# trnKhanh/medical-image-analysis

Hardware: AMD Instinct MI355X
Metric: training images/sec (whole node), UNet 512x512 1ch bs=32/GPU (higher is better)
Workload: dtype bf16; 1 GPU; UNet-2D channels [64, 128, 256, 512, 1024] 512x512 1ch, batch 32/GPU, instance norm, dropout 0.1, Dice+CE, Adam(wd 5e-4), clip 10 (cfg3); global_batch=32, parallelism=dp1

## Files before the change

include/mia_hip.h:

```cpp
#ifndef MIA_HIP_H
#define MIA_HIP_H
#include <stdint.h>
#ifdef __cplusplus
extern "C" {
#endif

#define MIA_F32 0
#define MIA_BF16 1

int mia_version(void);
const char* mia_last_error(void);

int mia_pack_weight(const float* src, void* dst, int dtype, int d0, int d1, int taps, int npad, int kpad,
                    int n_from_d0, void* stream);
int mia_pack_desc_bytes(void);
int mia_pack_weight_batch(const void* descs_dev, int count, int total_bricks, int max_taps, int dtype, void* stream);
int mia_relayout(const void* src, int src_dtype, void* dst, int dst_dtype, int n, int c, int64_t hw,
                 int64_t ssn, int64_t ssc, int64_t ssp, int64_t dsn, int64_t dsc, int64_t dsp, void* stream);
int mia_add(const void* a, const void* b, void* out, int dtype, int64_t n, void* stream);
int mia_dropout_mask(float* out, int64_t n, float keep, uint64_t seed, uint64_t offset, void* stream);
int mia_dropout_mask_dyn(float* out, int64_t n, float keep, const uint64_t* seed_base, uint64_t rel_offset, void* stream);
int mia_zero(void* p, int64_t bytes, void* stream);
int mia_gather_f32(const float* src, int64_t stride, float* dst, int n, void* stream);
int mia_colsum_workspace(int64_t p, int c);
// ... 16 lines not shown
#define MIA_CONV_FAM_FAST 1
#define MIA_CONV_FAM_S2_WIDE 2
#define MIA_CONV_FAM_CONV64 3
#define MIA_CONV_FAM_CONV64_DMA 4
#define MIA_CONV_FAM_CONV_BT 5
#define MIA_CONV_FAM_CONV_PW 6
#define MIA_CONV_FAM_NL 7
#define MIA_CONV_FAM_ACC 8
#define MIA_CONV_VAR_STATS 4
#define MIA_CONV_VAR_BIAS 8
int mia_conv_mma_family(int mode, int dtype, int c1, int c2, int o1, int o2, int npad, int kpad, int hout, int wout, int variant,
                        int split);
int mia_split_desc_bytes(void);
int mia_split_f16_batch(const void* descs_dev, int count, void* stream);
int mia_amax(const float* x, int64_t n, void* slot, int reset, void* stream);
int mia_widen_u8_i64(const void* src, void* dst, int64_t n, void* stream);
int mia_host_narrow_labels(const int64_t* src, uint8_t* dst, int64_t n, int threads);
int mia_host_copy(void* dst, const void* src, int64_t bytes, int threads);
int mia_amax_desc_bytes(void);
int mia_amax_batch(const void* descs_dev, int count, void* slots, void* stream);

int mia_conv_nl_supported(int mode, int dtype, int c1, int nout, int hout, int wout);
int mia_conv_mma_nl(int mode, int dtype, const void* y_in, int c1, const float* in_scale, const float* in_shift, float slope,
                    const void* wpack, int npad, int kpad, const float* bias, void* out, int nout, float* stat_partials,
                    int n, int hin, int win, int hout, int wout, void* stream);

int mia_conv_acc_supported(int mode, int dtype, int c1, int nout);
int mia_conv_mma_acc(int mode, int dtype, const void* in1, int c1, const void* wpack, int npad, int kpad, int flip_taps,
                     void* out_inout, int nout, int n, int hin, int win, int hout, int wout, const void* amax_in, const void* amax_w,
                     const void* wpack_split, void* stream);


int mia_stem_slabs(void);
int mia_stem_wgrad_workspace(int c0);
int mia_stem_fwd(const void* x, int x_dtype, const float* w, const float* bias, void* y, int dtype, float* stat_partials, int n,
                 int h, int wd, int c0, void* stream);
int mia_stem_wgrad(const void* x, int x_dtype, const void* dy, int dtype, float* workspace, float* grad, int n, int h, int wd,
                   int c0, int accumulate, void* stream);
int mia_stem_wgrad_fused(const void* x, int x_dtype, const void* dz, const void* y, int dtype, const float* scale,
                         const float* shift, const float* xa, const float* xb, const float* c1, const float* c2, float slope,
                         float* workspace, float* grad, int n, int h, int wd, int c0, int accumulate, void* stream);
int mia_stem_dgrad(const void* dy, int dtype, const float* w, float* dx, int n, int h, int wd, int c0, void* stream);

#define MIA_WGRAD_3S1 0
#define MIA_WGRAD_3S2 1
#define MIA_WGRAD_2S2 2
int mia_wgrad_target_blocks(int mode, int dtype);
int mia_wgrad_geometry(int mode, int dtype, int hy, int wy, int* tiles_y, int* tiles_x);
int mia_wgrad_plan(int mode, int dtype, int c1, int c2, int cdy, int npad, int hy, int* column_blocks, int* target_blocks, int* tile_h);
#define MIA_WGRAD_FAM_DMA96 0
#define MIA_WGRAD_FAM_BT 1
#define MIA_WGRAD_FAM_DMA 2
#define MIA_WGRAD_FAM_2WG 3
#define MIA_WGRAD_FAM_2WG_NL 4
#define MIA_WGRAD_FAM_TILE_FAST 5
#define MIA_WGRAD_FAM_F32_FAST 6
#define MIA_WGRAD_FAM_F32_NARROW 7
#define MIA_WGRAD_FAM_GENERIC 8
int mia_wgrad_family(int mode, int dtype, int c1, int c2, int cdy, int npad, int variant, int split);
int mia_conv_wgrad(int mode, int dtype, const void* x1, int c1, const void* x2, int c2, const void* dy, int cdy,
                   float* slabs, int ksplit, int npad, int kpad, int n, int hx, int wx, int hy, int wy, const void* amax_x1,
                   const void* amax_x2, const void* amax_dy, void* stream);
int mia_wgrad_nl_supported(int mode, int dtype, int c1, int cdy);
int mia_conv_wgrad_nl(int mode, int dtype, const void* y_in, int c1, const float* in_scale, const float* in_shift, float slope,
                      const void* dy, int cdy, float* slabs, int ksplit, int npad, int kpad, int n, int hx, int wx, int hy,
                      int wy, void* stream);
int mia_wgrad_reduce(const float* slabs, int ksplit, int taps, int npad, int kpad, float* grad, int nn, int kk,
                     int accumulate, void* stream);

#define MIA_NORM_INSTANCE 0
#define MIA_NORM_BATCH 1
int mia_norm_finalize(const float* partials, int n, int tiles, int c, int64_t hw, int mode, int training,
                      const float* drop_scale, const float* gamma, const float* beta, float eps, float momentum,
                      float* running_mean, float* running_var, long long* num_batches, float* xa, float* xb,
                      float* scale, float* shift, float* ysum, void* stream);
int mia_norm_stats(const void* y, int dtype, int n, int64_t hw, int c, int slabs, float* partials, void* stream);
int mia_norm_act_fwd(const void* y, void* z, int dtype, const float* scale, const float* shift, int n, int64_t hw, int c,
                     float slope, void* amax_out, void* stream);
int mia_norm_two_piece_ok(int dtype, int c);
int mia_norm_act_bwd(const void* dz, const void* dz2, const void* y, void* dy, int dtype, const float* scale, const float* shift,
                     const float* xa, const float* xb, const float* ysum, int n, int64_t hw, int c, int mode,
                     int fixed_stats, float slope, int slabs, float* partials, float* c1, float* c2, float* dgamma,
                     float* dbeta, float* dbias, int accumulate, void* amax_out, void* stream);
int mia_norm_bwd_sums(const void* dz, const void* dz2, const void* y, int dtype, const float* scale, const float* shift,
                      const float* xa, const float* xb, const float* ysum, int n, int64_t hw, int c, int mode,
                      int fixed_stats, float slope, int slabs, float* partials, float* c1, float* c2, float* dgamma,
                      float* dbeta, float* dbias, int accumulate, void* stream);

int mia_bn_sync_local_stats(const float* partials, int n, int tiles, int c, int64_t hw, const float* drop_scale, float* xa,
                            float* xb, float* local, void* stream);
int mia_norm_finalize_sync(const float* gathered, int world, int n, int c, int64_t hw, const float* drop_scale,
                           const float* gamma, const float* beta, float eps, float momentum, float* running_mean,
                           float* running_var, long long* num_batches, float* xa, float* xb, float* scale, float* shift,
                           float* ysum, void* stream);
int mia_norm_act_bwd_reduce(const void* dz, const void* dz2, const void* y, int dtype, const float* scale, const float* shift, const float* xa,
                            const float* xb, int n, int64_t hw, int c, float slope, int slabs, float* partials, float* c1,
                            float* c2, float* tot, void* stream);
int mia_norm_act_bwd_apply_sync(const void* dz, const void* dz2, const void* y, void* dy, int dtype, const float* scale, const float* shift,
                                const float* xa, const float* xb, const float* ysum, int n, int64_t hw, int c, float slope,
                                float* c1, float* c2, const float* group_tot, float* dgamma, float* dbeta, float* dbias,
                                int accumulate, void* amax_out, void* stream);

int mia_head_fwd(const void* x, int dtype, const float* w, const float* b, float* logits, int n, int64_t hw, int c0, int k1,
                 int64_t osn, int64_t osk, int64_t osp, void* stream);
int mia_head_bwd_workspace(int c0, int k1);
int mia_head_bwd(const float* dlogits, const void* x, int dtype, const float* w, void* dx, float* dw, float* db,
                 float* workspace, int n, int64_t hw, int c0, int k1, int64_t gsn, int64_t gsk, int64_t gsp, int accumulate,
                 void* stream);
#define MIA_LOSS_SOFTMAX 1
#define MIA_LOSS_DO_BG 2
#define MIA_LOSS_BATCH 4
#define MIA_LOSS_SQUARED 8
#define MIA_LOSS_DENSE 16
int mia_dice_ce_workspace(int nb, int k1, int slabs);
int mia_dice_ce_fwd(const float* logits, const long long* labels, int nb, int64_t hw, int k1, int64_t sn, int64_t sk,
                    int64_t sp, int flags, float smooth, float dice_w, float ce_w, int slabs, float* workspace, float* sums,
                    float* coef, float* out, int* bad_label, void* stream);
int mia_dice_ce_bwd(const float* logits, const long long* labels, const float* coef, const float* grad_out, float* dlogits,
                    int nb, int64_t hw, int k1, int64_t sn, int64_t sk, int64_t sp, int64_t gsn, int64_t gsk, int64_t gsp,
                    int flags, float dice_w, float ce_w, void* stream);

int mia_ds_loss_workspace(int nb, int k1, int slabs);
int mia_ds_loss_fwd(const float* z, const long long* labels, int nb, int h, int w, int factor, int k1, int64_t sn, int64_t sk,
                    int64_t sp, int flags, float smooth, float dice_w, float ce_w, int slabs, float* workspace, float* sums,
                    float* coef, float* out, int* bad_label, void* stream);
int mia_ds_loss_bwd(const float* z, const long long* labels, const float* coef, const float* grad_out, float* dz, int nb, int h,
                    int w, int factor, int k1, int64_t sn, int64_t sk, int64_t sp, int64_t gsn, int64_t gsk, int64_t gsp, int flags,
                    float dice_w, float ce_w, void* stream);

int mia_head_norm_eligible(int dtype, int n, int64_t hw, int c0, int k1);
int mia_head_norm_fwd(const void* y, int dtype, const float* scale, const float* shift, float slope, const float* w,
                      const float* b, float* logits, int n, int64_t hw, int c0, int k1, int64_t osn, int64_t osk, int64_t osp,
                      void* stream);
int mia_head_norm_wgrad(const float* dlogits, const void* y, int dtype, const float* scale, const float* shift, float slope,
                        float* dw, float* db, float* workspace, int n, int64_t hw, int c0, int k1, int64_t gsn, int64_t gsk,
                        int64_t gsp, int accumulate, void* stream);
int mia_norm_act_bwd_head(const float* dlogits, const float* w, int k1, int64_t gsn, int64_t gsk, int64_t gsp, const void* y,
                          void* dy, int dtype, const float* scale, const float* shift, const float* xa, const float* xb,
                          const float* ysum, int n, int64_t hw, int c, int mode, int fixed_stats, float slope, int slabs,
                          float* partials, float* c1, float* c2, float* dgamma, float* dbeta, float* dbias, int accumulate,
                          void* amax_out, void* stream);
int mia_head_w_supported(int dtype, int c, int k1);
int mia_norm_act_bwd_head_w(const float* dlogits, const float* w, int k1, int64_t gsn, int64_t gsk, int64_t gsp,
                            const void* y, void* dy, int dtype, const float* scale, const float* shift, const float* xa,
                            const float* xb, const float* ysum, int n, int64_t hw, int c, int mode, int fixed_stats,
                            float slope, int slabs, float* partials, float* c1, float* c2, float* dgamma, float* dbeta,
                            float* dbias, int accumulate, float* head_workspace, float* dw_head, float* db_head,
                            int accumulate_head, void* amax_out, void* stream);

#define MIA_SEGLOSS_SOFTMAX 1
#define MIA_SEGLOSS_DO_BG 2
#define MIA_SEGLOSS_BATCH 4
#define MIA_SEGLOSS_LABEL_U8 8
#define MIA_SEGLOSS_IGNORE 16
int mia_seg_loss_workspace(int nb, int k1, int slabs);
int mia_seg_loss_fwd(const float* logits, const void* labels, const float* class_w, int nb, int64_t hw, int k1, int64_t sn,
                     int64_t sk, int64_t sp, int flags, int64_t ignore_label, float smooth, float dice_w, float ce_w, int slabs,
                     float* workspace, float* coef, float* out, int64_t* counts, int* bad_label, void* stream);
int mia_seg_loss_bwd(const float* logits, const void* labels, const float* class_w, const float* coef, const float* grad_out,
                     float* dlogits, int nb, int64_t hw, int k1, int64_t sn, int64_t sk, int64_t sp, int64_t gsn, int64_t gsk,
                     int64_t gsp, int flags, int64_t ignore_label, void* stream);
int mia_topk_ce_workspace(int64_t n_pixels);
int mia_topk_ce_fwd(const float* logits, const void* labels, const float* class_w, int nb, int64_t hw, int k1, int64_t sn,
                    int64_t sk, int64_t sp, int flags, int64_t ignore_label, int64_t n_top, float* workspace, float* out,
                    int* bad_label, void* stream);
int mia_topk_ce_bwd(const float* logits, const void* labels, const float* class_w, const float* workspace, const float* grad_out,
// ... 162 lines not shown
```

medical-image-analysis_amd/csrc/norm.hip:

```cpp
#include "common.h"
#include "options.h"
#include <stdlib.h>

#define NORM_INSTANCE 0
#define NORM_BATCH 1

template <bool INST>
__global__ __launch_bounds__(1024) void norm_fwd_sum_kernel(const float* __restrict__ part, int tiles, int c, float* __restrict__ xa, float* __restrict__ xb,
                                    int64_t hw, const float* __restrict__ drop, const float* __restrict__ gamma,
                                    const float* __restrict__ beta, float eps, float* __restrict__ scale, float* __restrict__ shift,
                                    float* __restrict__ ysum) {
  __shared__ double sh1[16][17], sh2[16][17];
  const int cl = threadIdx.x & 15, tl = threadIdx.x >> 4;
  const int n = blockIdx.x, ch = blockIdx.y * 16 + cl;
  double s1 = 0.0, s2 = 0.0;
  if (ch < c) {
    typedef float f2_t __attribute__((ext_vector_type(2)));
    const f2_t* p = reinterpret_cast<const f2_t*>(part) + (size_t)n * tiles * c + ch;
    int t = tl;
    for (; t + 192 < tiles; t += 256) {
      const f2_t v0 = p[(size_t)t * c], v1 = p[(size_t)(t + 64) * c], v2 = p[(size_t)(t + 128) * c], v3 = p[(size_t)(t + 192) * c];
      s1 += (double)v0.x + (double)v1.x + (double)v2.x + (double)v3.x;
      s2 += (double)v0.y + (double)v1.y + (double)v2.y + (double)v3.y;
    }
// ... 289 lines not shown
  } while (0)

extern "C" int mia_norm_stats(const void* y, int dtype, int n, int64_t hw, int c, int slabs, float* partials, void* stream) {
  MIA_CHECK_ARG(y && partials && n > 0 && hw > 0 && c > 0 && slabs > 0, "mia_norm_stats: bad arguments");
  hipStream_t st = static_cast<hipStream_t>(stream);
  if (c % 32 == 0 && (reinterpret_cast<uintptr_t>(y) & 15) == 0 && (dtype == MIA_BF16 || dtype == MIA_F32)) {
    if (dtype == MIA_BF16)
      CRV(bf16_t, false, static_cast<const bf16_t*>(y), static_cast<const bf16_t*>(nullptr), static_cast<const bf16_t*>(nullptr), nullptr, nullptr, nullptr, nullptr, 0.f);
    else
      CRV(float, false, static_cast<const float*>(y), static_cast<const float*>(nullptr), static_cast<const float*>(nullptr), nullptr, nullptr, nullptr, nullptr, 0.f);
    MIA_LAUNCH_CHECK();
    return MIA_OK;
  }
  if (dtype == MIA_BF16)
    hipLaunchKernelGGL(norm_stats_kernel<bf16_t>, dim3(n * slabs, ceil_div(c, 256)), dim3(256), 512 * sizeof(float), st, static_cast<const bf16_t*>(y), hw, c, slabs, partials);
  else if (dtype == MIA_F32)
    hipLaunchKernelGGL(norm_stats_kernel<float>, dim3(n * slabs, ceil_div(c, 256)), dim3(256), 512 * sizeof(float), st, static_cast<const float*>(y), hw, c, slabs, partials);
  else { mia_set_error("mia_norm_stats: bad dtype"); return MIA_EARG; }
  MIA_LAUNCH_CHECK();
  return MIA_OK;
}

extern "C" int mia_amax(const float* x, int64_t n, void* slot, int reset, void* stream);
template <typename T> __device__ __forceinline__ void amax_fold(unsigned& m, const T* out) {
  if constexpr (sizeof(T) == 4) {
#pragma unroll
    for (int e = 0; e < Elem<T>::EPU; ++e) { const unsigned b = __builtin_bit_cast(unsigned, out[e]) & 0x7FFFFFFFu; m = b > m ? b : m; }
  }
}
__device__ __forceinline__ void amax_publish(unsigned m, unsigned* __restrict__ slot) {
  __shared__ unsigned blk;
  if (threadIdx.x == 0) blk = 0u;
  __syncthreads();
#pragma unroll
  for (int o = 32; o > 0; o >>= 1) { const unsigned t = (unsigned)__shfl_xor((int)m, o, 64); m = t > m ? t : m; }
  if ((threadIdx.x & 63) == 0 && m != 0u) atomicMax(&blk, m);
  __syncthreads();
  if (threadIdx.x == 0) {
    const unsigned b = blk;
    if (b > __hip_atomic_load(slot, __ATOMIC_RELAXED, __HIP_MEMORY_SCOPE_AGENT)) atomicMax(slot, b);
  }
}

template <typename T>
__global__ __launch_bounds__(256) void norm_act_fwd_stream_kernel(const T* __restrict__ y, T* __restrict__ z,
                                                                  const float* __restrict__ scale, const float* __restrict__ shift,
                                                                  int64_t hw, int c, int slabs, int upb, float slope,
                                                                  unsigned* __restrict__ amax) {
  constexpr int EPU = Elem<T>::EPU;
  const int n = blockIdx.x / slabs, s = blockIdx.x % slabs;
  const int lanes = 256 / upb;
  const int u = blockIdx.y * upb + threadIdx.x % upb, pl = threadIdx.x / upb;
  const bool live = u * EPU < c;
  if (!live && (sizeof(T) != 4 || amax == nullptr)) return;
  const int64_t per = (hw + slabs - 1) / slabs, r0 = s * per, r1 = live ? (r0 + per < hw ? r0 + per : hw) : r0;
  float sc[EPU], sf[EPU];
  unsigned am = 0;
#pragma unroll
  for (int e = 0; e < EPU; ++e) { sc[e] = live ? scale[(size_t)n * c + u * EPU + e] : 0.f; sf[e] = live ? shift[(size_t)n * c + u * EPU + e] : 0.f; }
  const size_t base = (size_t)n * hw * c + (size_t)u * EPU;
  auto body = [&](const u32x4& raw, int64_t r) {
    alignas(16) T in[EPU]; alignas(16) T out[EPU];
    *reinterpret_cast<u32x4*>(in) = raw;
#pragma unroll
    for (int e = 0; e < EPU; ++e) {
      const float v = sc[e] * Elem<T>::ld(in + e) + sf[e];
      out[e] = Elem<T>::cvt(v > 0.f ? v : v * slope);
    }
    amax_fold<T>(am, out);
    store_data_fence();
    *reinterpret_cast<u32x4*>(z + base + r * c) = *reinterpret_cast<const u32x4*>(out);
    store_data_pad();
  };
  auto ld = [&](int64_t rr) -> u32x4 { return *reinterpret_cast<const u32x4*>(y + base + rr * c); };
  int64_t r = r0 + pl;
  for (; r + 3 * lanes < r1; r += 4 * lanes) {
    const u32x4 a0 = ld(r), a1 = ld(r + lanes), a2 = ld(r + 2 * lanes), a3 = ld(r + 3 * lanes);
    body(a0, r); body(a1, r + lanes); body(a2, r + 2 * lanes); body(a3, r + 3 * lanes);
  }
  for (; r < r1; r += lanes) body(ld(r), r);
  if constexpr (sizeof(T) == 4) { if (amax != nullptr) amax_publish(am, amax); }
}

template <typename T, bool TWO = false>
__global__ __launch_bounds__(256) void norm_act_bwd_stream_kernel(const T* __restrict__ dz, const T* __restrict__ dz2,
                                                                  const T* __restrict__ y, T* __restrict__ dy,
                                                                  const float* __restrict__ scale, const float* __restrict__ shift,
                                                                  const float* __restrict__ xa, const float* __restrict__ xb,
                                                                  const float* __restrict__ c1, const float* __restrict__ c2,
                                                                  int64_t hw, int c, int slabs, int upb, float slope,
                                                                  unsigned* __restrict__ amax) {
  constexpr int EPU = Elem<T>::EPU;
  const int n = blockIdx.x / slabs, s = blockIdx.x % slabs;
  const int lanes = 256 / upb;
  const int u = blockIdx.y * upb + threadIdx.x % upb, pl = threadIdx.x / upb;
  const bool live = u * EPU < c;
  if (!live && (sizeof(T) != 4 || amax == nullptr)) return;
  const int64_t per = (hw + slabs - 1) / slabs, r0 = s * per, r1 = live ? (r0 + per < hw ? r0 + per : hw) : r0;
  float sc[EPU], sf[EPU], ka[EPU], kb[EPU];
  unsigned am = 0;
#pragma unroll
  for (int e = 0; e < EPU; ++e) {
    const size_t o = live ? (size_t)n * c + u * EPU + e : 0;
    sc[e] = scale[o]; sf[e] = shift[o];
    ka[e] = -sc[e] * c2[o] * xa[o];
    kb[e] = -sc[e] * (c1[o] + c2[o] * xb[o]);
  }
  const size_t base = (size_t)n * hw * c + (size_t)u * EPU;
  auto body = [&](const u32x4& graw, const u32x4& g2raw, const u32x4& yraw, int64_t r) {
    alignas(16) T gin[EPU]; alignas(16) T g2in[EPU]; alignas(16) T yin[EPU]; alignas(16) T out[EPU];
    *reinterpret_cast<u32x4*>(gin) = graw;
    *reinterpret_cast<u32x4*>(g2in) = g2raw;
    *reinterpret_cast<u32x4*>(yin) = yraw;
#pragma unroll
    for (int e = 0; e < EPU; ++e) {
      const float yv = Elem<T>::ld(yin + e);
      float g = Elem<T>::ld(gin + e);
      if (TWO) g += Elem<T>::ld(g2in + e);
      out[e] = Elem<T>::cvt(norm_bwd_dy(g, yv, sc[e], sf[e], ka[e], kb[e], slope));
    }
    amax_fold<T>(am, out);
    store_data_fence();
    *reinterpret_cast<u32x4*>(dy + base + r * c) = *reinterpret_cast<const u32x4*>(out);
    store_data_pad();
  };
  const u32x4 zero = u32x4{0u, 0u, 0u, 0u};
  auto ld = [&](const T* ptr, int64_t r) { return *reinterpret_cast<const u32x4*>(ptr + base + r * c); };
  int64_t r = r0 + pl;
  for (; r + lanes < r1; r += 2 * lanes) {
    const u32x4 g0 = ld(dz, r), h0 = TWO ? ld(dz2, r) : zero, y0 = ld(y, r);
    const u32x4 g1 = ld(dz, r + lanes), h1 = TWO ? ld(dz2, r + lanes) : zero, y1 = ld(y, r + lanes);
    body(g0, h0, y0, r); body(g1, h1, y1, r + lanes);
  }
  for (; r < r1; r += lanes) body(ld(dz, r), TWO ? ld(dz2, r) : zero, ld(y, r), r);
  if constexpr (sizeof(T) == 4) { if (amax != nullptr) amax_publish(am, amax); }
}

static void stream_geometry(int n, int64_t hw, int c, int epu, int* slabs, int* upb, int* gy) {
  const int upp = c / epu;
  int ub = 1;
  while (ub < upp && ub < 64) ub <<= 1;
  *upb = ub;
  *gy = (upp + ub - 1) / ub;
  const int lanes = 256 / ub;
  const int target = mia_options().stream_blocks;
  int64_t sl = target / ((int64_t)n * *gy);
  const int64_t maxsl = hw / (lanes * 8) > 0 ? hw / (lanes * 8) : 1;
  if (sl > maxsl) sl = maxsl;
  if (sl < 1) sl = 1;
  *slabs = (int)sl;
}

template <typename T, bool VEC>
__global__ void norm_act_fwd_kernel(const T* __restrict__ y, T* __restrict__ z, const float* __restrict__ scale,
                                    const float* __restrict__ shift, int64_t hw, int c, int64_t total_units, float slope) {
  constexpr int EPU = VEC ? Elem<T>::EPU : 1;
  const int upp = c / EPU;
  for (int64_t u = (int64_t)blockIdx.x * blockDim.x + threadIdx.x; u < total_units; u += (int64_t)gridDim.x * blockDim.x) {
    const int64_t pix = u / upp;
    const int ch = (int)(u - pix * upp) * EPU;
    const int n = (int)(pix / hw);
    const float* sc = scale + (size_t)n * c + ch;
    const float* sf = shift + (size_t)n * c + ch;
    if constexpr (VEC) {
      const u32x4 raw = *reinterpret_cast<const u32x4*>(y + u * EPU);
      alignas(16) T in[EPU]; alignas(16) T out[EPU];
      *reinterpret_cast<u32x4*>(in) = raw;
#pragma unroll
      for (int e = 0; e < EPU; ++e) {
        const float v = sc[e] * Elem<T>::ld(in + e) + sf[e];
        out[e] = Elem<T>::cvt(v > 0.f ? v : v * slope);
      }
      *reinterpret_cast<u32x4*>(z + u * EPU) = *reinterpret_cast<const u32x4*>(out);
    } else {
      const float v = sc[0] * Elem<T>::ld(y + u) + sf[0];
      Elem<T>::st(z + u, v > 0.f ? v : v * slope);
    }
  }
}

extern "C" int mia_norm_act_fwd(const void* y, void* z, int dtype, const float* scale, const float* shift, int n, int64_t hw,
                                int c, float slope, void* amax_out, void* stream) {
  MIA_CHECK_ARG(y && z && scale && shift && n > 0 && hw > 0 && c > 0, "mia_norm_act_fwd: bad arguments");
  if (dtype != MIA_F32) amax_out = nullptr;
  const int epu = dtype == MIA_BF16 ? 8 : 4;
  const bool vec = (c % epu == 0) && ((reinterpret_cast<uintptr_t>(y) | reinterpret_cast<uintptr_t>(z)) & 15) == 0;
  const int64_t units = (int64_t)n * hw * (vec ? c / epu : c);
  const int blocks = (int)((units + 255) / 256 < 16384 ? (units + 255) / 256 : 16384);
  hipStream_t st = static_cast<hipStream_t>(stream);
// ... 130 lines not shown
  }
}

template <typename T, bool VEC>
__global__ void norm_act_bwd_apply_kernel(const T* __restrict__ dz, const T* __restrict__ y, T* __restrict__ dy,
                                          const float* __restrict__ scale, const float* __restrict__ shift,
                                          const float* __restrict__ xa, const float* __restrict__ xb,
                                          const float* __restrict__ c1, const float* __restrict__ c2, int64_t hw, int c,
                                          int64_t total_units, float slope) {
  constexpr int EPU = VEC ? Elem<T>::EPU : 1;
  const int upp = c / EPU;
  for (int64_t u = (int64_t)blockIdx.x * blockDim.x + threadIdx.x; u < total_units; u += (int64_t)gridDim.x * blockDim.x) {
    const int64_t pix = u / upp;
    const int ch = (int)(u - pix * upp) * EPU;
    const size_t o = (size_t)(pix / hw) * c + ch;
    alignas(16) T gin[EPU]; alignas(16) T yin[EPU]; alignas(16) T out[EPU];
    if constexpr (VEC) {
      *reinterpret_cast<u32x4*>(gin) = *reinterpret_cast<const u32x4*>(dz + u * EPU);
      *reinterpret_cast<u32x4*>(yin) = *reinterpret_cast<const u32x4*>(y + u * EPU);
    } else { gin[0] = dz[u]; yin[0] = y[u]; }
#pragma unroll
    for (int e = 0; e < EPU; ++e) {
      const float yv = Elem<T>::ld(yin + e);
      float g = Elem<T>::ld(gin + e);
      if (!(scale[o + e] * yv + shift[o + e] > 0.f)) g *= slope;
      const float xh = xa[o + e] * yv + xb[o + e];
      out[e] = Elem<T>::cvt(scale[o + e] * (g - c1[o + e] - xh * c2[o + e]));
    }
    if constexpr (VEC) *reinterpret_cast<u32x4*>(dy + u * EPU) = *reinterpret_cast<const u32x4*>(out);
    else dy[u] = out[0];
  }
}

static bool bwd_vec_ok(const void* dz, const void* y, const void* dy, int dtype, int c) {
  const int epu = dtype == MIA_BF16 ? 8 : 4;
  return (c % epu == 0) &&
         ((reinterpret_cast<uintptr_t>(y) | reinterpret_cast<uintptr_t>(dz) | reinterpret_cast<uintptr_t>(dy)) & 15) == 0;
}

struct NormBwd {
  const void *dz, *dz2, *y; void* dy; int dtype;
  const float *scale, *shift, *xa, *xb, *ysum;
  int n; int64_t hw; int c, mode, fixed_stats; float slope; int slabs;
  float *partials, *c1, *c2, *dgamma, *dbeta, *dbias; int accumulate;
  void* amax_out; hipStream_t st;
};

extern "C" int mia_norm_two_piece_ok(int dtype, int c) { return (dtype == MIA_BF16 || dtype == MIA_F32) && c % 32 == 0; }

static int bwd_check(const char* who, const NormBwd& p, bool tensors, bool need_partials, bool need_grads) {
  MIA_CHECK_ARG(tensors && p.scale && p.shift && p.xa && p.xb && p.c1 && p.c2 && (!need_partials || p.partials) &&
                (!need_grads || (p.dgamma && p.dbeta)), "%s: null pointer", who);
  MIA_CHECK_ARG(p.n > 0 && p.hw > 0 && p.c > 0 && (!need_partials || p.slabs > 0), "%s: bad shape", who);
  MIA_CHECK_ARG(p.dtype == MIA_BF16 || p.dtype == MIA_F32, "%s: bad dtype", who);
  MIA_CHECK_ARG(p.dz2 == nullptr || (p.c % 32 == 0 && bwd_vec_ok(p.dz, p.y, p.dy, p.dtype, p.c) && (reinterpret_cast<uintptr_t>(p.dz2) & 15) == 0),
                "%s: two-piece gradient needs c %% 32 == 0 and aligned tensors", who);
  return MIA_OK;
}

static void bwd_reduce_launch(const NormBwd& p) {
  const int n = p.n, c = p.c, slabs = p.slabs;
  const int64_t hw = p.hw; float* partials = p.partials; hipStream_t st = p.st;
  const bool vec = bwd_vec_ok(p.dz, p.y, nullptr, p.dtype, c);
#define RD(T) hipLaunchKernelGGL(norm_act_bwd_reduce_kernel<T>, dim3(n * slabs, ceil_div(c, 256)), dim3(256), 512 * sizeof(float), st,   \
                                 static_cast<const T*>(p.dz), static_cast<const T*>(p.y), p.scale, p.shift, p.xa, p.xb, hw, c, slabs, \
                                 p.slope, partials)
#define RDV(T) CRV(T, true, static_cast<const T*>(p.dz), static_cast<const T*>(p.y), static_cast<const T*>(p.dz2), p.scale, p.shift, p.xa, p.xb, p.slope)
  if (vec && c % 32 == 0) { if (p.dtype == MIA_BF16) RDV(bf16_t); else RDV(float); }
  else if (p.dtype == MIA_BF16) RD(bf16_t); else RD(float);
#undef RDV
#undef RD
}

static void bwd_finalize_launch(const NormBwd& p, bool producer_parts = false, const float* group_tot = nullptr) {
  const bool own = !producer_parts && group_tot == nullptr;
  const bool inline_sums = own && (int64_t)p.n * p.slabs <= 1024;
  if (group_tot == nullptr && !inline_sums)
    hipLaunchKernelGGL(norm_bwd_sum_kernel, dim3(p.n, ceil_div(p.c, 16)), dim3(256), 0, p.st, p.partials, p.slabs, p.c, p.c1, p.c2);
  hipLaunchKernelGGL(norm_bwd_finalize_kernel, dim3(ceil_div(p.c, 16)), dim3(256), 0, p.st, p.n, p.c, p.hw, p.mode, p.fixed_stats,
                     p.scale, p.xa, p.xb, p.ysum, p.c1, p.c2, p.dgamma, p.dbeta, p.dbias, p.accumulate, group_tot,
                     inline_sums ? p.partials : nullptr, own ? p.slabs : 0);
}

static void bwd_apply_launch(const NormBwd& p) {
  void* amax_out = p.dtype == MIA_F32 ? p.amax_out : nullptr;
  const int epu = p.dtype == MIA_BF16 ? 8 : 4;
  const bool vec = bwd_vec_ok(p.dz, p.y, p.dy, p.dtype, p.c);
  const int64_t units = (int64_t)p.n * p.hw * (vec ? p.c / epu : p.c);
  const int blocks = (int)((units + 255) / 256 < 16384 ? (units + 255) / 256 : 16384);
#define AP(T, V) hipLaunchKernelGGL((norm_act_bwd_apply_kernel<T, V>), dim3(blocks), dim3(256), 0, p.st,                   \
                                    static_cast<const T*>(p.dz), static_cast<const T*>(p.y), static_cast<T*>(p.dy), p.scale, p.shift, \
                                    p.xa, p.xb, p.c1, p.c2, p.hw, p.c, units, p.slope)
  if (vec) {
    int sl, upb, gy;
    stream_geometry(p.n, p.hw, p.c, epu, &sl, &upb, &gy);
#define BS(T, TWOF) hipLaunchKernelGGL((norm_act_bwd_stream_kernel<T, TWOF>), dim3(p.n * sl, gy), dim3(256), 0, p.st, static_cast<const T*>(p.dz), \
                                       static_cast<const T*>(p.dz2), static_cast<const T*>(p.y), static_cast<T*>(p.dy), p.scale, p.shift, p.xa, p.xb, \
                                       p.c1, p.c2, p.hw, p.c, sl, upb, p.slope, static_cast<unsigned*>(amax_out))
    if (p.dtype == MIA_BF16) { if (p.dz2) BS(bf16_t, true); else BS(bf16_t, false); }
    else { if (p.dz2) BS(float, true); else BS(float, false); }
#undef BS
  } else {
    if (p.dtype == MIA_BF16) AP(bf16_t, false);
    else AP(float, false);
    if (amax_out) (void)mia_amax(static_cast<const float*>(p.dy), (int64_t)p.n * p.hw * p.c, amax_out, 0, p.st);
  }
#undef AP
}

extern "C" int mia_norm_act_bwd(const void* dz, const void* dz2, const void* y, void* dy, int dtype, const float* scale, const float* shift,
                                const float* xa, const float* xb, const float* ysum, int n, int64_t hw, int c, int mode,
                                int fixed_stats, float slope, int slabs, float* partials, float* c1, float* c2, float* dgamma,
                                float* dbeta, float* dbias, int accumulate, void* amax_out, void* stream) {
  const NormBwd p{dz, dz2, y, dy, dtype, scale, shift, xa, xb, ysum, n, hw, c, mode, fixed_stats, slope, slabs, partials, c1, c2,
                  dgamma, dbeta, dbias, accumulate, amax_out, static_cast<hipStream_t>(stream)};
  if (int e = bwd_check("mia_norm_act_bwd", p, dz && y && dy, true, true)) return e;
  bwd_reduce_launch(p);
  bwd_finalize_launch(p);
  bwd_apply_launch(p);
  MIA_LAUNCH_CHECK();
  return MIA_OK;
}

extern "C" int mia_norm_bwd_sums(const void* dz, const void* dz2, const void* y, int dtype, const float* scale, const float* shift,
                                 const float* xa, const float* xb, const float* ysum, int n, int64_t hw, int c, int mode,
                                 int fixed_stats, float slope, int slabs, float* partials, float* c1, float* c2, float* dgamma,
                                 float* dbeta, float* dbias, int accumulate, void* stream) {
  const NormBwd p{dz, dz2, y, nullptr, dtype, scale, shift, xa, xb, ysum, n, hw, c, mode, fixed_stats, slope, slabs, partials, c1, c2,
                  dgamma, dbeta, dbias, accumulate, nullptr, static_cast<hipStream_t>(stream)};
  if (int e = bwd_check("mia_norm_bwd_sums", p, dz && y, true, true)) return e;
  bwd_reduce_launch(p);
  bwd_finalize_launch(p);
  MIA_LAUNCH_CHECK();
  return MIA_OK;
}

#ifdef MIA_EXPERIMENTS
extern "C" int mia_norm_act_bwd_pre(const void* dz, const void* y, void* dy, int dtype, const float* scale, const float* shift,
                                    const float* xa, const float* xb, const float* ysum, int n, int64_t hw, int c, int mode,
                                    int fixed_stats, float slope, int parts, const float* partials, float* c1, float* c2,
                                    float* dgamma, float* dbeta, float* dbias, int accumulate, void* amax_out, void* stream) {
  const NormBwd p{dz, nullptr, y, dy, dtype, scale, shift, xa, xb, ysum, n, hw, c, mode, fixed_stats, slope, parts,
                  const_cast<float*>(partials), c1, c2, dgamma, dbeta, dbias, accumulate, amax_out, static_cast<hipStream_t>(stream)};
  if (int e = bwd_check("mia_norm_act_bwd_pre", p, true, true, true)) return e;
  MIA_CHECK_ARG(dy == nullptr || (dz && y), "mia_norm_act_bwd_pre: the apply pass needs dz and y");
  bwd_finalize_launch(p, true);
  if (dy != nullptr) bwd_apply_launch(p);
  MIA_LAUNCH_CHECK();
  return MIA_OK;
}

#endif

__global__ void bn_bwd_local_tot_kernel(int n_img, int c, int64_t hw, const float* __restrict__ c1, const float* __restrict__ c2,
                                        float* __restrict__ tot) {
  __shared__ double sh1[16][17], sh2[16][17];
  const int cl = threadIdx.x & 15, tl = threadIdx.x >> 4;
  const int ch = blockIdx.x * 16 + cl;
  double tg = 0.0, tgx = 0.0;
  if (ch < c)
    for (int n = tl; n < n_img; n += 16) { tg += c1[(size_t)n * c + ch]; tgx += c2[(size_t)n * c + ch]; }
  sh1[tl][cl] = tg; sh2[tl][cl] = tgx;
  __syncthreads();
  if (tl == 0 && ch < c) {
    tg = 0.0; tgx = 0.0;
    for (int j = 0; j < 16; ++j) { tg += sh1[j][cl]; tgx += sh2[j][cl]; }
    tot[ch] = (float)tg; tot[c + ch] = (float)tgx; tot[2 * c + ch] = (float)((double)n_img * (double)hw);
  }
}

extern "C" int mia_norm_act_bwd_reduce(const void* dz, const void* dz2, const void* y, int dtype, const float* scale, const float* shift,
                                       const float* xa, const float* xb, int n, int64_t hw, int c, float slope, int slabs,
                                       float* partials, float* c1, float* c2, float* tot, void* stream) {
  const NormBwd p{dz, dz2, y, nullptr, dtype, scale, shift, xa, xb, nullptr, n, hw, c, NORM_BATCH, 0, slope, slabs, partials, c1, c2,
                  nullptr, nullptr, nullptr, 0, nullptr, static_cast<hipStream_t>(stream)};
  if (int e = bwd_check("mia_norm_act_bwd_reduce", p, dz && y && tot, true, false)) return e;
  bwd_reduce_launch(p);
  hipLaunchKernelGGL(norm_bwd_sum_kernel, dim3(n, ceil_div(c, 16)), dim3(256), 0, p.st, partials, slabs, c, c1, c2);
  hipLaunchKernelGGL(bn_bwd_local_tot_kernel, dim3(ceil_div(c, 16)), dim3(256), 0, p.st, n, c, hw, c1, c2, tot);
  MIA_LAUNCH_CHECK();
  return MIA_OK;
}

extern "C" int mia_norm_act_bwd_apply_sync(const void* dz, const void* dz2, const void* y, void* dy, int dtype, const float* scale,
                                           const float* shift, const float* xa, const float* xb, const float* ysum, int n,
                                           int64_t hw, int c, float slope, float* c1, float* c2, const float* group_tot,
                                           float* dgamma, float* dbeta, float* dbias, int accumulate, void* amax_out, void* stream) {
  const NormBwd p{dz, dz2, y, dy, dtype, scale, shift, xa, xb, ysum, n, hw, c, NORM_BATCH, 0, slope, 0, nullptr, c1, c2,
                  dgamma, dbeta, dbias, accumulate, amax_out, static_cast<hipStream_t>(stream)};
  if (int e = bwd_check("mia_norm_act_bwd_apply_sync", p, dz && y && dy && group_tot, false, true)) return e;
  bwd_finalize_launch(p, false, group_tot);
  bwd_apply_launch(p);
  MIA_LAUNCH_CHECK();
  return MIA_OK;
}

template <typename T, int K1, int CG, bool HWG = false>
__global__ __launch_bounds__(256) void colreduce_head_kernel(const float* __restrict__ dl, const float* __restrict__ w,
                                                             const T* __restrict__ y, const float* __restrict__ scale,
                                                             const float* __restrict__ shift, const float* __restrict__ xa,
                                                             const float* __restrict__ xb, int hw, int c, int slabs, float slope,
                                                             int64_t gsn, int64_t gsp, int64_t gsk, float* __restrict__ part, float* __restrict__ wpart) {
// ... 242 lines not shown
```

medical-image-analysis_amd/mia_hip/ops.py:

```python
from __future__ import annotations

import ctypes
import math
from typing import Optional, Tuple

import torch

from . import (BF16, CONV_G1, CONV_G2S2, CONV_G3S1, CONV_G3S2, CONV_T2S2, CONV_T3S2, F32, LOSS_BATCH, LOSS_DO_BG,
               LOSS_DENSE, LOSS_SOFTMAX, LOSS_SQUARED, NORM_BATCH, NORM_INSTANCE, REGLOSS_BATCH, REGLOSS_DO_BG, REGLOSS_IGNORE,
               REGLOSS_INDEX, REGLOSS_TARGET_U8, SEGLOSS_BATCH, SEGLOSS_DO_BG, SEGLOSS_IGNORE,
               SEGLOSS_LABEL_U8, SEGLOSS_SOFTMAX, WGRAD_2S2, WGRAD_3S1, WGRAD_3S2, MiaError, call, lib)

LRELU_SLOPE = 0.01
_c_int, _c_float, _c_i64 = ctypes.c_int, ctypes.c_float, ctypes.c_int64


def _p(t: Optional[torch.Tensor]):
    return None if t is None else ctypes.c_void_p(t.data_ptr())


def _stream():
    return ctypes.c_void_p(torch.cuda.current_stream().cuda_stream)


# ... 589 lines not shown


_BN_TRACKING = True


class no_bn_tracking:

    def __enter__(self):
        global _BN_TRACKING
        self._was, _BN_TRACKING = _BN_TRACKING, False

    def __exit__(self, *exc):
        global _BN_TRACKING
        _BN_TRACKING = self._was
        return False


def _norm_finalize(ctx, cfg: NormCfg, stats, gamma, beta, y) -> torch.Tensor:
    n, h, w, cout = y.shape
    hw = h * w
    coefs = torch.empty((5, n, cout), device=y.device, dtype=torch.float32)
    ctx.sync = sync = cfg.sync if (cfg.sync is not None and cfg.mode == NORM_BATCH and cfg.training and cfg.sync.world > 1) else None
    track = _BN_TRACKING or not cfg.training
    rmean, rvar, nbatch = (cfg.running_mean, cfg.running_var, cfg.num_batches) if track else (None, None, None)
    if sync is None:
        call("mia_norm_finalize", _p(stats), n, 0 if stats is None else stats.shape[1], cout, _c_i64(hw), cfg.mode, int(cfg.training),
             _p(cfg.drop_scale), _p(gamma.detach()), _p(beta.detach()), _c_float(cfg.eps), _c_float(cfg.momentum),
             _p(rmean), _p(rvar), _p(nbatch), _p(coefs[0]), _p(coefs[1]), _p(coefs[2]),
             _p(coefs[3]), _p(coefs[4]), _stream())
        return coefs
    local = torch.empty((3, cout), device=stats.device, dtype=torch.float32)
    call("mia_bn_sync_local_stats", _p(stats), n, stats.shape[1], cout, _c_i64(hw), _p(cfg.drop_scale), _p(coefs[0]),
         _p(coefs[1]), _p(local), _stream())
    gathered = sync.all_gather(local)
    call("mia_norm_finalize_sync", _p(gathered), sync.world, n, cout, _c_i64(hw), _p(cfg.drop_scale), _p(gamma.detach()),
         _p(beta.detach()), _c_float(cfg.eps), _c_float(cfg.momentum), _p(rmean), _p(rvar),
         _p(nbatch), _p(coefs[0]), _p(coefs[1]), _p(coefs[2]), _p(coefs[3]), _p(coefs[4]), _stream())
    return coefs


def _norm_act_fwd(y, scale, shift, slope) -> torch.Tensor:
    n, h, w, c = y.shape
    z = torch.empty_like(y)
    call("mia_norm_act_fwd", _p(y), _p(z), _dt(y), _p(scale), _p(shift), n, _c_i64(h * w), c, _c_float(slope), _p(_amax_new(z)), _stream())
    return z


class LazyAct:
    __slots__ = ("y", "coefs", "slope")

    def __init__(self, y, coefs, slope):
        self.y, self.coefs, self.slope = y, coefs, slope

    @property
    def shape(self):
        return self.y.shape

    @property
    def dtype(self):
        return self.y.dtype

    @property
    def device(self):
        return self.y.device

    def materialize(self) -> torch.Tensor:
        return LazyMaterializeFn.apply(self.y, self.coefs, self.slope)


class LazyMaterializeFn(torch.autograd.Function):

    @staticmethod
    def forward(ctx, y, coefs, slope):
        return _norm_act_fwd(y, coefs[2], coefs[3], slope)

    @staticmethod
    def backward(ctx, dz):
        return dz, None, None


FUSE_HEAD_W = __import__('os').environ.get('MIA_FUSE_HEAD_W', '1') != '0'
FUSE_STEM_BWD = __import__('os').environ.get('MIA_FUSE_STEM_BWD', '1') != '0'
FUSE_NL = __import__('os').environ.get('MIA_FUSE_NL', '1') != '0'


def nl_supported(dtype, cin: int, cout: int, h: int, w: int, train: bool) -> bool:
    if not FUSE_NL or dtype != torch.bfloat16:
        return False
    if not lib().mia_conv_nl_supported(CONV_G3S1, BF16, cin, cout, h, w):
        return False
    return (not train) or bool(lib().mia_wgrad_nl_supported(WGRAD_3S1, BF16, cin, cout))


class _NormBwd:

    def __init__(self, y, coefs, mode, fixed, slope, dests=None):
        self.y, self.coefs, self.mode, self.fixed, self.slope = y, coefs, mode, fixed, slope
        n, h, w, c = y.shape
        self.dtype, self.n, self.hw, self.c, self.slabs = _dt(y), n, h * w, c, _slabs_for(h * w)
        self.part = torch.empty((n, self.slabs, c, 2), device=y.device, dtype=torch.float32)
        self.cc = torch.empty((2, n, c), device=y.device, dtype=torch.float32)
        dgb = torch.empty((3, c), device=y.device, dtype=torch.float32)
        got = (None,) * 3 if dests is None else [grad_dest(p) for p in dests]
        self.dgamma, self.dbeta, self.dbias = (dgb[i] if g is None else g for i, g in enumerate(got))

    def _run(self, slabs, part):
        k = self.coefs
        return (_p(k[2]), _p(k[3]), _p(k[0]), _p(k[1]), _p(None if self.fixed else k[4]), self.n, _c_i64(self.hw), self.c, self.mode,
                int(self.fixed), _c_float(self.slope), slabs, _p(part), _p(self.cc[0]), _p(self.cc[1]), _p(self.dgamma),
                _p(self.dbeta), _p(self.dbias), 0)

    def plain(self, dz, dz2, dy) -> None:
        call("mia_norm_act_bwd", _p(dz), _p(dz2), _p(self.y), _p(dy), self.dtype, *self._run(self.slabs, self.part),
             _p(_amax_new(dy)), _stream())

    def sums(self, dz, dz2) -> None:
        call("mia_norm_bwd_sums", _p(dz), _p(dz2), _p(self.y), self.dtype, *self._run(self.slabs, self.part), _stream())

    def pre(self, parts, dz, dy) -> None:
        call("mia_norm_act_bwd_pre", _p(None if dy is None else dz), _p(None if dy is None else self.y), _p(dy), self.dtype,
             *self._run(parts.shape[1], parts), _p(None if dy is None else _amax_new(dy)), _stream())

    def synced(self, sync: BatchSync, dz, dz2, dy) -> None:
        k, cc = self.coefs, self.cc
        tot = torch.empty((3, self.c), device=self.y.device, dtype=torch.float32)
        call("mia_norm_act_bwd_reduce", _p(dz), _p(dz2), _p(self.y), self.dtype, _p(k[2]), _p(k[3]), _p(k[0]), _p(k[1]), self.n,
             _c_i64(self.hw), self.c, _c_float(self.slope), self.slabs, _p(self.part), _p(cc[0]), _p(cc[1]), _p(tot), _stream())
        sync.all_reduce_sum(tot)
        call("mia_norm_act_bwd_apply_sync", _p(dz), _p(dz2), _p(self.y), _p(dy), self.dtype, _p(k[2]), _p(k[3]), _p(k[0]), _p(k[1]),
             _p(k[4]), self.n, _c_i64(self.hw), self.c, _c_float(self.slope), _p(cc[0]), _p(cc[1]), _p(tot), _p(self.dgamma),
             _p(self.dbeta), _p(self.dbias), 0, _p(_amax_new(dy)), _stream())

    def run(self, dz, dz2, sync, on_load: bool) -> Optional[torch.Tensor]:
        pre = _take_cr(dz) if (dz2 is None and sync is None) else None
        dy = None if on_load else torch.empty_like(self.y)
        if pre is not None:
            self.pre(pre, dz, dy)
        elif sync is not None:
            self.synced(sync, dz, dz2, dy)
        elif on_load:
            self.sums(dz, dz2)
        else:
            self.plain(dz, dz2, dy)
        return dy

    def head(self, dl, st, w2, dy, entry="mia_norm_act_bwd_head", extra=()) -> None:
        call(entry, _p(dl), _p(w2), w2.shape[0], _c_i64(st[0]), _c_i64(st[1]), _c_i64(st[2]), _p(self.y), _p(dy), self.dtype,
             *self._run(self.slabs, self.part), *extra, _p(_amax_new(dy)), _stream())

    def head_w(self, dl, st, w2, dy, ws, dwh, dbh) -> None:
        self.head(dl, st, w2, dy, "mia_norm_act_bwd_head_w", (_p(ws), _p(dwh), _p(dbh), 0))


def _block_wgrad(nb: _NormBwd, x1, x2, weight, stride: int, nl, dy, stem: bool = False, dz=None, dz2=None) -> torch.Tensor:
    cout, cin = weight.shape[:2]
    y, k = nb.y, nb.coefs
    if not stem:
        dw = conv_wgrad(WGRAD_3S2 if stride == 2 else WGRAD_3S1, x1, x2, dy, weight.shape, cout, cin, out=grad_dest(weight), nl=nl)
    else:
        if dy is None and dz2 is not None:
            dz = dz + dz2
        ws = torch.empty(lib().mia_stem_wgrad_workspace(cout), device=y.device, dtype=torch.float32)
        dw = grad_dest(weight)
        if dw is None:
            dw = torch.empty(weight.shape, device=y.device, dtype=torch.float32)
        if dy is None:
            call("mia_stem_wgrad_fused", _p(x1), _dt(x1), _p(dz), _p(y), nb.dtype, _p(k[2]), _p(k[3]), _p(k[0]), _p(k[1]),
                 _p(nb.cc[0]), _p(nb.cc[1]), _c_float(nb.slope), _p(ws), _p(dw), nb.n, y.shape[1], y.shape[2], cout, 0, _stream())
        else:
            call("mia_stem_wgrad", _p(x1), _dt(x1), _p(dy), nb.dtype, _p(ws), _p(dw), nb.n, y.shape[1], y.shape[2], cout, 0, _stream())
    return dw


def _stem_dgrad(dy, weight, x1) -> torch.Tensor:
    n, h, w, cout = dy.shape
    w2 = weight.detach().reshape(cout, 9)
    if not w2.is_contiguous():
        w2 = w2.contiguous()
    dx = torch.empty((n, h, w, 1), device=dy.device, dtype=torch.float32)
    call("mia_stem_dgrad", _p(dy), _dt(dy), _p(w2), _p(dx), n, h, w, cout, _stream())
    return dx if x1.dtype == torch.float32 else cast_nhwc(dx, x1.dtype)


def _block_dgrad(x1, x2, weight, dy, stride: int, nl, dup_in: bool, need1: bool, need2: bool):
    dx1 = dx2 = None
    dtype = _dt(dy)
    n, ho, wo, cout = dy.shape
    c1, cin = x1.shape[3], weight.shape[1]
    wb, npad, kpad = pack_cache(weight).get(weight, dtype, n_from_d0=False)
    split = c1 if x2 is not None else None
    other = _take_acc(x1) if (stride == 2 and x2 is None and dup_in) else None
    if other is not None and lib().mia_conv_acc_supported(CONV_T3S2, dtype, cout, cin):
        amw = getattr(wb, "_mia_amax", None) if _split_ok(dy, n * ho * wo * cout * cin) else None
        call("mia_conv_mma_acc", CONV_T3S2, dtype, _p(dy), cout, _p(wb), npad, kpad, 0, _p(other), cin, n, ho, wo,
             x1.shape[1], x1.shape[2], _p(None if amw is None else amax_slot(dy)), _p(None if amw is None else amw[0]),
# ... 1356 lines not shown
```

Before: 792.5 images/sec.

## Fold instance-norm backward finalize into the apply streaming kernel

Adds a fused backward path for instance norm. The separate finalize kernel that turns slab partials into per-channel means and parameter gradients is removed, and the apply kernel recomputes these per block from the partials, with block n==0 also reducing dgamma/dbeta/dbias. This saves one kernel launch and a round trip through global memory per norm layer, in exchange for redundant partial reductions in every block. It also sets a launch-bounds occupancy hint that may constrain registers. Large n*slabs cases fall back to a separate sum kernel.

```diff
diff --git a/include/mia_hip.h b/include/mia_hip.h
--- a/include/mia_hip.h
+++ b/include/mia_hip.h
@@ -122,6 +122,10 @@
                      const float* xa, const float* xb, const float* ysum, int n, int64_t hw, int c, int mode,
                      int fixed_stats, float slope, int slabs, float* partials, float* c1, float* c2, float* dgamma,
                      float* dbeta, float* dbias, int accumulate, void* amax_out, void* stream);
+int mia_norm_act_bwd_fold(const void* dz, const void* dz2, const void* y, void* dy, int dtype, const float* scale, const float* shift,
+                          const float* xa, const float* xb, const float* ysum, int n, int64_t hw, int c, int mode,
+                          int fixed_stats, float slope, int slabs, float* partials, float* c1, float* c2, float* dgamma,
+                          float* dbeta, float* dbias, int accumulate, float* sums, void* amax_out, void* stream);
 int mia_norm_bwd_sums(const void* dz, const void* dz2, const void* y, int dtype, const float* scale, const float* shift,
                       const float* xa, const float* xb, const float* ysum, int n, int64_t hw, int c, int mode,
                       int fixed_stats, float slope, int slabs, float* partials, float* c1, float* c2, float* dgamma,
diff --git a/medical-image-analysis_amd/csrc/norm.hip b/medical-image-analysis_amd/csrc/norm.hip
--- a/medical-image-analysis_amd/csrc/norm.hip
+++ b/medical-image-analysis_amd/csrc/norm.hip
@@ -395,19 +395,92 @@
   if constexpr (sizeof(T) == 4) { if (amax != nullptr) amax_publish(am, amax); }
 }
 
-template <typename T, bool TWO = false>
-__global__ __launch_bounds__(256) void norm_act_bwd_stream_kernel(const T* __restrict__ dz, const T* __restrict__ dz2,
+struct NormBwdFold {
+  const float* part; int pslabs;
+  const float* sums;
+  const float* ysum; float *c1, *c2, *dgamma, *dbeta, *dbias; int n_img, accumulate;
+};
+
+__device__ __forceinline__ void fold_sums(const NormBwdFold& f, int n, int c, int ch, float& sg, float& sgx) {
+  if (f.part == nullptr) { sg = f.sums[(size_t)n * c + ch]; sgx = f.sums[((size_t)f.n_img + n) * c + ch]; return; }
+  typedef float f2_t __attribute__((ext_vector_type(2)));
+  const f2_t* p = reinterpret_cast<const f2_t*>(f.part) + (size_t)n * f.pslabs * c + ch;
+  double s1 = 0.0, s2 = 0.0;
+#pragma unroll 2
+  for (int t = 0; t < f.pslabs; ++t) { const f2_t v = p[(size_t)t * c]; s1 += v.x; s2 += v.y; }
+  sg = (float)s1; sgx = (float)s2;
+}
+
+__device__ __forceinline__ void fold_param_grads(const NormBwdFold& f, int c, int64_t hw, int ch_lo, int ch_hi, int s, int slabs,
+                                                 const float* __restrict__ scale, const float* __restrict__ xa,
+                                                 const float* __restrict__ xb) {
+  __shared__ double sh1[16][17], sh2[16][17], sh3[16][17];
+  const int cl = threadIdx.x & 15, tl = threadIdx.x >> 4;
+  const double M = (double)hw;
+  for (int g0 = ch_lo + 16 * s; g0 < ch_hi; g0 += 16 * slabs) {
+    const int ch = g0 + cl;
+    double tg = 0.0, tgx = 0.0;
+    if (ch < ch_hi)
+      for (int n = tl; n < f.n_img; n += 16) {
+        float fg, fgx;
+        fold_sums(f, n, c, ch, fg, fgx);
+        tg += fg; tgx += fgx;
+      }
+    sh1[tl][cl] = tg; sh2[tl][cl] = tgx;
+    double tb = 0.0;
+    if (f.dbias && ch < ch_hi)
+      for (int n = tl; n < f.n_img; n += 16) {
+        const size_t idx = (size_t)n * c + ch;
+        float fg, fgx;
+        fold_sums(f, n, c, ch, fg, fgx);
+        const double sg = fg, sgx = fgx;
+        const double m1 = sg / M, m2 = sgx / M;
+        const double sxh = f.ysum ? (double)xa[idx] * f.ysum[idx] + M * xb[idx] : 0.0;
+        tb += (double)scale[idx] * (sg - M * m1 - m2 * sxh);
+      }
+    sh3[tl][cl] = tb;
+    __syncthreads();
+    if (tl == 0 && ch < ch_hi) {
+      tg = 0.0; tgx = 0.0; tb = 0.0;
+      for (int j = 0; j < 16; ++j) { tg += sh1[j][cl]; tgx += sh2[j][cl]; tb += sh3[j][cl]; }
+      f.dgamma[ch] = f.accumulate ? f.dgamma[ch] + (float)tgx : (float)tgx;
+      f.dbeta[ch] = f.accumulate ? f.dbeta[ch] + (float)tg : (float)tg;
+      if (f.dbias) f.dbias[ch] = f.accumulate ? f.dbias[ch] + (float)tb : (float)tb;
+    }
+    __syncthreads();
+  }
+}
+
+template <typename T, bool TWO = false, bool FOLD = false>
+__global__ __launch_bounds__(256, FOLD ? 7 : 1) void norm_act_bwd_stream_kernel(const T* __restrict__ dz, const T* __restrict__ dz2,
                                                                   const T* __restrict__ y, T* __restrict__ dy,
                                                                   const float* __restrict__ scale, const float* __restrict__ shift,
                                                                   const float* __restrict__ xa, const float* __restrict__ xb,
                                                                   const float* __restrict__ c1, const float* __restrict__ c2,
                                                                   int64_t hw, int c, int slabs, int upb, float slope,
-                                                                  unsigned* __restrict__ amax) {
+                                                                  unsigned* __restrict__ amax, NormBwdFold fold) {
   constexpr int EPU = Elem<T>::EPU;
   const int n = blockIdx.x / slabs, s = blockIdx.x % slabs;
   const int lanes = 256 / upb;
   const int u = blockIdx.y * upb + threadIdx.x % upb, pl = threadIdx.x / upb;
   const bool live = u * EPU < c;
+  __shared__ float means[FOLD ? 2 : 1][FOLD ? 64 * EPU : 1];
+  if constexpr (FOLD) {
+    const int cw = upb * EPU, cb = blockIdx.y * cw;
+    const double M = (double)hw;
+    for (int j = threadIdx.x; j < cw; j += 256) {
+      const int ch = cb + j;
+      if (ch < c) {
+        float fg, fgx;
+        fold_sums(fold, n, c, ch, fg, fgx);
+        const float m1 = (float)((double)fg / M), m2 = (float)((double)fgx / M);
+        means[0][j] = m1; means[1][j] = m2;
+        if (s == 0) { fold.c1[(size_t)n * c + ch] = m1; fold.c2[(size_t)n * c + ch] = m2; }
+      } else { means[0][j] = 0.f; means[1][j] = 0.f; }
+    }
+    if (n == 0) fold_param_grads(fold, c, hw, cb, cb + cw < c ? cb + cw : c, s, slabs, scale, xa, xb);
+    __syncthreads();
+  }
   if (!live && (sizeof(T) != 4 || amax == nullptr)) return;
   const int64_t per = (hw + slabs - 1) / slabs, r0 = s * per, r1 = live ? (r0 + per < hw ? r0 + per : hw) : r0;
   float sc[EPU], sf[EPU], ka[EPU], kb[EPU];
@@ -415,9 +488,10 @@
 #pragma unroll
   for (int e = 0; e < EPU; ++e) {
     const size_t o = live ? (size_t)n * c + u * EPU + e : 0;
+    const float m1 = FOLD ? means[0][(threadIdx.x % upb) * EPU + e] : c1[o], m2 = FOLD ? means[1][(threadIdx.x % upb) * EPU + e] : c2[o];
     sc[e] = scale[o]; sf[e] = shift[o];
-    ka[e] = -sc[e] * c2[o] * xa[o];
-    kb[e] = -sc[e] * (c1[o] + c2[o] * xb[o]);
+    ka[e] = -sc[e] * m2 * xa[o];
+    kb[e] = -sc[e] * (m1 + m2 * xb[o]);
   }
   const size_t base = (size_t)n * hw * c + (size_t)u * EPU;
   auto body = [&](const u32x4& graw, const u32x4& g2raw, const u32x4& yraw, int64_t r) {
@@ -714,7 +788,12 @@
                      inline_sums ? p.partials : nullptr, own ? p.slabs : 0);
 }
 
-static void bwd_apply_launch(const NormBwd& p) {
+static bool bwd_fold_ok(const NormBwd& p, const float* sums) {
+  return p.mode == NORM_INSTANCE && !p.fixed_stats && bwd_vec_ok(p.dz, p.y, p.dy, p.dtype, p.c) &&
+         ((int64_t)p.n * p.slabs <= 1024 || sums != nullptr);
+}
+
+static void bwd_apply_launch(const NormBwd& p, bool fold = false, const float* sums = nullptr) {
   void* amax_out = p.dtype == MIA_F32 ? p.amax_out : nullptr;
   const int epu = p.dtype == MIA_BF16 ? 8 : 4;
   const bool vec = bwd_vec_ok(p.dz, p.y, p.dy, p.dtype, p.c);
@@ -726,11 +805,15 @@
   if (vec) {
     int sl, upb, gy;
     stream_geometry(p.n, p.hw, p.c, epu, &sl, &upb, &gy);
-#define BS(T, TWOF) hipLaunchKernelGGL((norm_act_bwd_stream_kernel<T, TWOF>), dim3(p.n * sl, gy), dim3(256), 0, p.st, static_cast<const T*>(p.dz), \
+    const bool long_sums = (int64_t)p.n * p.slabs > 1024;
+    const NormBwdFold f{fold && !long_sums ? p.partials : nullptr, p.slabs, sums, p.ysum, p.c1, p.c2, p.dgamma, p.dbeta, p.dbias, p.n, p.accumulate};
+#define BS(T, TWOF, FOLDF) hipLaunchKernelGGL((norm_act_bwd_stream_kernel<T, TWOF, FOLDF>), dim3(p.n * sl, gy), dim3(256), 0, p.st, static_cast<const T*>(p.dz), \
                                        static_cast<const T*>(p.dz2), static_cast<const T*>(p.y), static_cast<T*>(p.dy), p.scale, p.shift, p.xa, p.xb, \
-                                       p.c1, p.c2, p.hw, p.c, sl, upb, p.slope, static_cast<unsigned*>(amax_out))
-    if (p.dtype == MIA_BF16) { if (p.dz2) BS(bf16_t, true); else BS(bf16_t, false); }
-    else { if (p.dz2) BS(float, true); else BS(float, false); }
+                                       p.c1, p.c2, p.hw, p.c, sl, upb, p.slope, static_cast<unsigned*>(amax_out), f)
+#define BSF(T, TWOF) do { if (fold) BS(T, TWOF, true); else BS(T, TWOF, false); } while (0)
+    if (p.dtype == MIA_BF16) { if (p.dz2) BSF(bf16_t, true); else BSF(bf16_t, false); }
+    else { if (p.dz2) BSF(float, true); else BSF(float, false); }
+#undef BSF
 #undef BS
   } else {
     if (p.dtype == MIA_BF16) AP(bf16_t, false);
@@ -750,6 +833,28 @@
   bwd_reduce_launch(p);
   bwd_finalize_launch(p);
   bwd_apply_launch(p);
+  MIA_LAUNCH_CHECK();
+  return MIA_OK;
+}
+
+extern "C" int mia_norm_act_bwd_fold(const void* dz, const void* dz2, const void* y, void* dy, int dtype, const float* scale,
+                                     const float* shift, const float* xa, const float* xb, const float* ysum, int n, int64_t hw, int c,
+                                     int mode, int fixed_stats, float slope, int slabs, float* partials, float* c1, float* c2,
+                                     float* dgamma, float* dbeta, float* dbias, int accumulate, float* sums, void* amax_out,
+                                     void* stream) {
+  const NormBwd p{dz, dz2, y, dy, dtype, scale, shift, xa, xb, ysum, n, hw, c, mode, fixed_stats, slope, slabs, partials, c1, c2,
+                  dgamma, dbeta, dbias, accumulate, amax_out, static_cast<hipStream_t>(stream)};
+  if (int e = bwd_check("mia_norm_act_bwd_fold", p, dz && y && dy, true, true)) return e;
+  bwd_reduce_launch(p);
+  if (bwd_fold_ok(p, sums)) {
+    const bool long_sums = (int64_t)n * slabs > 1024;
+    if (long_sums)
+      hipLaunchKernelGGL(norm_bwd_sum_kernel, dim3(n, ceil_div(c, 16)), dim3(256), 0, p.st, partials, slabs, c, sums, sums + (size_t)n * c);
+    bwd_apply_launch(p, true, long_sums ? sums : nullptr);
+  } else {
+    bwd_finalize_launch(p);
+    bwd_apply_launch(p);
+  }
   MIA_LAUNCH_CHECK();
   return MIA_OK;
 }
diff --git a/medical-image-analysis_amd/mia_hip/ops.py b/medical-image-analysis_amd/mia_hip/ops.py
--- a/medical-image-analysis_amd/mia_hip/ops.py
+++ b/medical-image-analysis_amd/mia_hip/ops.py
@@ -695,6 +695,7 @@
 FUSE_HEAD_W = __import__('os').environ.get('MIA_FUSE_HEAD_W', '1') != '0'
 FUSE_STEM_BWD = __import__('os').environ.get('MIA_FUSE_STEM_BWD', '1') != '0'
 FUSE_NL = __import__('os').environ.get('MIA_FUSE_NL', '1') != '0'
+FOLD_FINALIZE = __import__('os').environ.get('MIA_FOLD_FINALIZE', '1') != '0'
 
 
 def nl_supported(dtype, cin: int, cout: int, h: int, w: int, train: bool) -> bool:
@@ -724,6 +725,11 @@
                 _p(self.dbeta), _p(self.dbias), 0)
 
     def plain(self, dz, dz2, dy) -> None:
+        if FOLD_FINALIZE:
+            sums = torch.empty((2, self.n, self.c), device=dy.device, dtype=torch.float32) if self.n * self.slabs > 1024 else None
+            call("mia_norm_act_bwd_fold", _p(dz), _p(dz2), _p(self.y), _p(dy), self.dtype, *self._run(self.slabs, self.part),
+                 _p(sums), _p(_amax_new(dy)), _stream())
+            return
         call("mia_norm_act_bwd", _p(dz), _p(dz2), _p(self.y), _p(dy), self.dtype, *self._run(self.slabs, self.part),
              _p(_amax_new(dy)), _stream())
 
```

Result: no change. 795.4 images/sec (median of 6 runs) (+0.4%).
